# armadaproject/armada

Hardware: NVIDIA H100
Metric: job-placements/sec per scheduling round; 100k nodes x 1M jobs (higher is better)
Workload: dtype int64+f64

## Files before the change

### armada_b200/csrc/armada_dev.h

```cpp
#pragma once
#include <stdint.h>
#ifndef ARMADA_EMU
#include <vector_types.h>
#endif

#include "armada_b200.h"

#define ARMADA_DEV_MAX_QUEUES 128
#define ARMADA_DEV_MAX_SLOTS 22
#define ARMADA_DEV_VARIANTS (1 + ARMADA_MAX_AWAY)

struct DevCfg {
  int32_t D, R, PL, PC, Q, C, T, S, rows;
  uint32_t N, J, G;
  int32_t indexed_resource[ARMADA_MAX_RESOURCES];
  int64_t res_scale[ARMADA_MAX_RESOURCES];
  int32_t key_shift[ARMADA_MAX_RESOURCES];
  int32_t res_key_shift[ARMADA_MAX_RESOURCES];
  int32_t res_key_width[ARMADA_MAX_RESOURCES];
  int32_t node_bits;
  int32_t key_total_bits;
  int32_t key_width[ARMADA_MAX_RESOURCES];
  unsigned long long key_guard;
  int32_t swar_ok;
  int32_t cls_global;
  int32_t exact;
  int64_t index_res[ARMADA_MAX_RESOURCES];
  int32_t collect_excl;
  int32_t k32_ok;
  int32_t priorities[ARMADA_MAX_PRIORITIES];
  ArmadaPriorityClass pcs[ARMADA_MAX_PRIORITY_CLASSES];
  int64_t total_resources[ARMADA_MAX_RESOURCES];
  double drf_mult[ARMADA_MAX_RESOURCES];
  int64_t max_to_schedule[ARMADA_MAX_RESOURCES];
  uint8_t has_round_limit, protect_uncapped, prefer_large, disable_home, disable_away, disable_gang_away,
      global_inf, _pad;
  double protected_fraction;
  uint32_t max_lookback, disallowed_mask;
  double global_tokens;
  int64_t global_burst;
  int32_t max_slots, sw, tw;
  int32_t win_w;
  uint32_t off_cls, off_win, off_touched, off_slot, off_skey, off_srow, off_ssc, off_sgpos, off_hb_key, off_hb_row, off_hb_sc,
      off_ring, off_bt_k0, off_bt_k1, off_bt_id;
  int32_t bt_wq;
  int32_t bt_np;
  uint32_t uni_V;
  uint32_t floating_mask;
  int32_t floating_configured;
  int64_t floating_limit[ARMADA_MAX_RESOURCES];
};

struct DevPtrs {
  const int64_t* node_total;
  const int64_t* node_allocatable;
  const uint32_t* node_sclass;
  const uint8_t* node_flags;
  const int64_t* class_req_raw;
  const int64_t* class_req_node;
  const uint32_t* class_pc;
  const uint32_t* class_row;
  const uint8_t* class_key_valid;
  const double* class_cost;
  const uint4* q_rec;
  uint4* ev_rec;
  const uint32_t* static_match;
  unsigned char* cls_glob;
// ... 109 lines not shown
```

### armada_b200/csrc/armada_host.inc

```

#define CUDA_TRY(expr)                                                                     \
  do {                                                                                     \
    cudaError_t _e = (expr);                                                               \
    if (_e != cudaSuccess) {                                                               \
      g_last_error = std::string(#expr) + ": " + cudaGetErrorString(_e);                   \
      return ARMADA_E_CUDA;                                                                \
    }                                                                                      \
  } while (0)

#ifdef ARMADA_EMU
static std::recursive_mutex& emu_mutex() {
  static std::recursive_mutex m;
  return m;
}
#define ARMADA_EMU_SERIAL std::lock_guard<std::recursive_mutex> emu_lock_(emu_mutex())
#else
#define ARMADA_EMU_SERIAL ((void)0)
#endif

template <class T>
struct PinnedVec {
  T* p = nullptr;
  size_t n = 0, cap = 0;
  PinnedVec() = default;
// ... 579 lines not shown
    off = align16(off + 4 * S);
    cfg.bt_wq = 0;
    cfg.bt_np = 0;
    cfg.off_bt_k0 = cfg.off_bt_k1 = cfg.off_bt_id = (uint32_t)off;
    int wq_cap = exact ? 0 : 64;
    if (const char* e = getenv("ARMADA_BT_WQ"))
      if (!exact) wq_cap = std::max(8, atoi(e));
    for (int wq = 64; wq >= 8; wq >>= 1) {
      if ((size_t)wq * Q > 4096 || wq > wq_cap) continue;
      size_t np = 2;
      while (np < (size_t)wq * Q) np <<= 1;
      size_t need = 2 * (8 + 8 + 2 + 2) * np + 64;
      if (off + need + 16 <= (size_t)dev_smem) {
        cfg.bt_wq = wq;
        cfg.bt_np = (int32_t)np;
        cfg.off_bt_k0 = (uint32_t)off;
        cfg.off_bt_k1 = (uint32_t)(off + 8 * np);
        off = align16(off + 2 * 16 * np);
        cfg.off_bt_id = (uint32_t)off;
        off = align16(off + 2 * 2 * 2 * np);
        break;
      }
    }
    r->smem_bytes = off + 16;
    if (timing)
      fprintf(stderr,
              "smem layout: %zu bytes (header %zu, batch buffers at %u, %d items per queue per batch, np %d, %d slots)"
              " exact %d swar_ok %d k32_ok %d key_total_bits %d node_bits %d bt_wq %d\n",
              r->smem_bytes, sizeof(SmemHdr), cfg.off_bt_k0, cfg.bt_wq, cfg.bt_np, cfg.max_slots, cfg.exact, cfg.swar_ok, cfg.k32_ok,
              cfg.key_total_bits, cfg.node_bits, cfg.bt_wq);
    if (r->smem_bytes > (size_t)dev_smem) return fail_status(ARMADA_E_UNSUPPORTED, "shared-memory layout does not fit");
    CUDA_TRY(cudaFuncSetAttribute(k_schedule_pass<1>, cudaFuncAttributeMaxDynamicSharedMemorySize, dev_smem));
    CUDA_TRY(cudaFuncSetAttribute(k_schedule_pass<2>, cudaFuncAttributeMaxDynamicSharedMemorySize, dev_smem));
    CUDA_TRY(cudaFuncSetAttribute(k_schedule_pass<3>, cudaFuncAttributeMaxDynamicSharedMemorySize, dev_smem));
    CUDA_TRY(cudaFuncSetAttribute(k_schedule_pass<4>, cudaFuncAttributeMaxDynamicSharedMemorySize, dev_smem));
    CUDA_TRY(cudaFuncSetAttribute(k_schedule_pass<8>, cudaFuncAttributeMaxDynamicSharedMemorySize, dev_smem));
  }

  lap("domain+layout");
  r->node_perm.assign(N, 0);
  r->node_inv.assign(N, 0);
  for (uint32_t n = 0; n < N; ++n) {
    r->node_perm[in->node_id_rank[n]] = n;
    r->node_inv[n] = in->node_id_rank[n];
  }
  std::vector<int64_t> h_total((size_t)D * N), h_alloc((size_t)D * N);
  std::vector<uint32_t> h_sclass(N);
  std::vector<uint8_t> h_flags(N);
  for (uint32_t dn = 0; dn < N; ++dn) {
    uint32_t e = r->node_perm[dn];
    h_sclass[dn] = in->node_static_class[e];
    h_flags[dn] = in->node_flags[e];
    for (uint32_t d = 0; d < D; ++d) {
// ... 400 lines not shown
  DA(excl, cfg.collect_excl ? (size_t)J * ARMADA_EXCLUDED_KINDS : 16);
  DA(undo_log, 5 * (3 * (size_t)J + 16));
  DA(ev_rec, J);
  DA(fp_avail, (size_t)D * N);
  DA(fp_epoch, N);
  DA(fp_head, N);
  DA(fp_next, J);
  DA(fp_bad, N);
  DA(nl_start, (size_t)N + 1);
  DA(nl_item, J);
  DA(nl_pos, J);
  DA(nver, N);
  DA(fc_ver, 16 * (size_t)N);
  DA(bver, (N + 255) / 256 + 1);
  DA(fc_bver, 8 * ((size_t)(N + 255) / 256 + 1));
  DA(fc_bmax, 8 * ((size_t)(N + 255) / 256 + 1));
  DA(q_alloc, (size_t)Q * D);
  DA(q_alloc_pc, (size_t)Q * PC * D);
  DA(q_fair, (size_t)Q * 3);
  DA(q_tokens, Q);
  DA(s_scheduled, D);
  DA(s_evicted, D);
  DA(s_counts, 8);
  DA(stats, 48);
  {
    void* dp = nullptr;
    CUDA_TRY(cudaHostGetDevicePointer(&dp, r->h_dbg, 0));
    P.dbg_host = (uint32_t*)dp;
  }
  st = r->dalloc(&r->d_state, J);
  if (st) return st;
  st = r->dalloc(&r->d_method, J);
  if (st) return st;
  st = r->dalloc(&r->d_reason, J);
  if (st) return st;
  st = r->dalloc(&r->d_node, J);
  if (st) return st;
  st = r->dalloc(&r->d_sched_at, J);
  if (st) return st;
  st = r->dalloc(&r->d_preempted_at, J);
  if (st) return st;
  st = r->dalloc(&r->d_evict_queue, Q);
  if (st) return st;
  st = r->dalloc(&r->d_oversub, N);
  if (st) return st;
  st = r->dalloc(&r->d_hist, 256 * (size_t)grid_for(std::max<uint32_t>(std::max(J, N), 1), RS_THREADS * RS_ITEMS) + 1024);
  if (st) return st;
// ... 198 lines not shown
    CUDA_TRY(cudaEventRecord(r->evp[3], s));
    launches += 1;
  }
  ARMADA_LAUNCH(k_finalize, gj, 256, 0, s, c, P, r->d_state, r->d_node, r->d_sched_at, r->d_preempted_at, r->d_method, r->d_reason);
  launches += 1;
  CUDA_TRY(cudaEventRecord(r->ev1, s));
  CUDA_TRY(cudaGetLastError());
  {
    cudaError_t e = cudaStreamSynchronize(s);
    if (e != cudaSuccess) {
      std::string msg = std::string("cudaStreamSynchronize: ") + cudaGetErrorString(e);
      if (r->h_dbg && r->h_dbg[0]) {
        msg += "; device watchdog: spin loop " + std::to_string(r->h_dbg[0]) + " in warp " + std::to_string(r->h_dbg[1]) + " wr=" + std::to_string(r->h_dbg[3]) + " rd=";
        for (int i = 0; i < 12; ++i) msg += std::to_string(r->h_dbg[4 + i]) + ",";
        msg += " bt_prog=";
        for (int i = 0; i < 12; ++i) msg += std::to_string(r->h_dbg[20 + i]) + ",";
        msg += " pl_ready=" + std::to_string(r->h_dbg[36]) + " pl_chain=" + std::to_string(r->h_dbg[37]) + " pl_home=" + std::to_string(r->h_dbg[38]) + " iters=" + std::to_string(r->h_dbg[39]);
      }
      g_last_error = msg;
      return ARMADA_E_CUDA;
    }
  }
  long long counts[8];
  unsigned long long dstats[48];
  CUDA_TRY(cudaMemcpy(counts, P.s_counts, sizeof(counts), cudaMemcpyDeviceToHost));
  CUDA_TRY(cudaMemcpy(dstats, P.stats, sizeof(dstats), cudaMemcpyDeviceToHost));
  if (counts[5] == 100) return fail_status(ARMADA_E_DEADLINE, "the round did not finish within its time budget; nothing was committed");
  if (counts[5] != 0) return fail_status(ARMADA_E_INTERNAL, "device invariant violated, code " + std::to_string(counts[5]));
  float ms = 0;
  CUDA_TRY(cudaEventElapsedTime(&ms, r->ev0, r->ev1));
  r->stats = ArmadaRoundStats{};
  if (getenv("ARMADA_PRINT_STATS"))
    fprintf(stderr,
            "armada stats: kernel_cycles=%llu startup=%llu pipeline_runs=%llu chain_busy=%llu chain_wait=%llu epilogue=%llu precreate=%llu first_batch_wait=%llu "
            "after_chain_wait=%llu failed_iters=%llu failed_cycles=%llu fair_query_cycles=%llu level_scan_cycles=%llu evicted_rebind_cycles=%llu\n",
            dstats[5], dstats[6], dstats[7], dstats[24], dstats[25], dstats[16 + 7], dstats[32], dstats[33], dstats[34], dstats[35], dstats[36], dstats[37],
            dstats[38], dstats[39]);
  if (getenv("ARMADA_PRINT_STATS"))
    fprintf(stderr,
            "armada general loop: wait_index_warps=%llu ring_full=%llu select_queued=%llu (n=%llu) bind_queued=%llu fair_victims=%llu iteration_prologue=%llu\n",
            dstats[40], dstats[41], dstats[42], dstats[46], dstats[43], dstats[44], dstats[45]);
  r->stats.loop_iterations = dstats[0];
  r->stats.probes = dstats[1];
  r->stats.placements = dstats[2];
  r->stats.fair_preemption_scans = dstats[3];
  r->stats.tree_rescans = dstats[4];
  for (int i = 0; i < 8; ++i) r->stats.phase_cycles[i] = dstats[8 + i];
  for (int i = 0; i < 8; ++i) r->stats.batch_cycles[i] = dstats[16 + i];
  for (int i = 0; i < 8; ++i) r->stats.batch_debug[i] = dstats[24 + i];
  r->stats.evicted_pass1 = e1;
  r->stats.evicted_pass2 = e2;
  r->stats.gpu_launches = launches;
  r->stats.device_ms = ms;
  {
    float p1 = 0, p2 = 0;
    CUDA_TRY(cudaEventElapsedTime(&p1, r->evp[0], r->evp[1]));
    if (e2 > 0) CUDA_TRY(cudaEventElapsedTime(&p2, r->evp[2], r->evp[3]));
    r->stats.schedule_pass_ms = p1 + p2;
  }
  if (stats) *stats = r->stats;
  r->ran = true;
  return ARMADA_OK;
}

// ... 193 lines not shown
```

### armada_b200/csrc/armada_pass.inc

```

#define g_c (H->env_c)
#define g_p (H->env_p)
#define g_a (H->env_a)

#define PASS_WARPS 16
#define PASS_THREADS (PASS_WARPS * 32)
#define IDX_WARPS 15
#define CTL_WARP (PASS_WARPS - 1)
#define IDX_OWNERS (IDX_WARPS - 1)
#define WIN 32
#define WIN_TARGET 12
#define WIN_LOW 4
#define MSG_CAP 32
#define TLOG_CAP 32

enum { MSG_EXIT = 0, MSG_UPDATE0 = 1, MSG_NEWSLOT = 2, MSG_SCAN = 3, MSG_BATCH = 4, MSG_SUCC = 5, MSG_FAIR = 6 };
#define BT_RING 32

#define REC_EVICTED 0x80000000u
#define REC_GANG 0x40000000u
#define REC_QEV 0x20000000u
#define REC_GS 0x10000000u
#define REC_GSL 0x08000000u
#define REC_CLS_MASK 0x00FFFFFFu
// ... 127 lines not shown
  uint32_t bt_lim[2];
  uint32_t cmask[8];
  uint32_t sc_mask[32];
  uint32_t bt_lastpos[2][ARMADA_DEV_MAX_QUEUES];
  uint32_t bt_apc[2][ARMADA_DEV_MAX_QUEUES];
  uint32_t bt_njobs[2][ARMADA_DEV_MAX_QUEUES];
  uint32_t pl_extra;
  uint32_t pl_cut, pl_skip;
  uint4 gang_rec;
  uint32_t gang_cons[64];
  uint32_t bt_fh[ARMADA_DEV_MAX_SLOTS];
  uint32_t grp_of[32];
  uint32_t grp_diff[32];
  int grp_ns;
  unsigned long long t_runs;
  unsigned long long tl[8];
  uint32_t grp_resume[32];
  uint32_t grp_first[32];
  uint32_t bt_lazy;
  unsigned long long slot_preq[32];
  uint32_t slot_okp;
  unsigned long long slot_py[32];
  uint4 cand_scr[32];
  unsigned long long bt_fk[ARMADA_DEV_MAX_SLOTS];
  unsigned long long seq_base;
  uint32_t bt_cool, bt_cool_len, bt_batches;
  int bt_precreated;
  unsigned long long bt_cyc[8];
  unsigned long long bt_dbg[8];
  BtRes bt_ring[BT_RING];
  unsigned long long prof[8];
  int error;
  unsigned long long deadline_ns;
};

struct Views {
  ClassRec* cls;
  uint4* win;
  uint32_t* touched;
  SlotHdr* slot;
  unsigned long long* skey;
  int64_t* srow;
  uint32_t* ssc;
  uint32_t* sgpos;
  unsigned long long* hb_key;
  int64_t* hb_row;
  uint32_t* hb_sc;
  Msg* ring;
  unsigned long long* bt_k0;
  unsigned long long* bt_k1;
  uint16_t* bt_id;
};

__device__ __forceinline__ Views make_views(const DevCfg& c, unsigned char* smem_raw) {
  Views V;
  V.cls = c.cls_global ? (ClassRec*)((SmemHdr*)smem_raw)->env_p.cls_glob : (ClassRec*)(smem_raw + c.off_cls);
  V.win = (uint4*)(smem_raw + c.off_win);
  V.touched = (uint32_t*)(smem_raw + c.off_touched);
  V.slot = (SlotHdr*)(smem_raw + c.off_slot);
  V.skey = (unsigned long long*)(smem_raw + c.off_skey);
  V.srow = (int64_t*)(smem_raw + c.off_srow);
  V.ssc = (uint32_t*)(smem_raw + c.off_ssc);
  V.sgpos = (uint32_t*)(smem_raw + c.off_sgpos);
  V.hb_key = (unsigned long long*)(smem_raw + c.off_hb_key);
  V.hb_row = (int64_t*)(smem_raw + c.off_hb_row);
  V.hb_sc = (uint32_t*)(smem_raw + c.off_hb_sc);
  V.ring = (Msg*)(smem_raw + c.off_ring);
  V.bt_k0 = (unsigned long long*)(smem_raw + c.off_bt_k0);
  V.bt_k1 = (unsigned long long*)(smem_raw + c.off_bt_k1);
  V.bt_id = (uint16_t*)(smem_raw + c.off_bt_id);
  return V;
}

#ifdef ARMADA_EMU
#define ARMADA_SMEM_BASE (emu::M().dyn_smem)
#else
extern __shared__ __align__(16) unsigned char armada_smem[];
#define ARMADA_SMEM_BASE armada_smem
#endif
#define H ((SmemHdr*)ARMADA_SMEM_BASE)
#define V (make_views(g_c, ARMADA_SMEM_BASE))
#define nodemask ((1ull << g_c.node_bits) - 1ull)

#define DEXACT(DM) ((DM) <= 4)

#define PROF_BEGIN long long _t0 = clock64()
#define PROF_END(i)                                   \
  do {                                                \
    if (lane_id() == 0) H->prof[i] += clock64() - _t0; \
  } while (0)

__device__ __forceinline__ unsigned long long armada_now_ns() {
#ifdef ARMADA_EMU
// ... 207 lines not shown
        if (dg < sh.cursor) sh.cursor = dg;
        sh.wm = min_u64(sh.wm, dk);
      } else {
        sh.lostmin = min_u64(sh.lostmin, dk);
      }
    }
    __syncwarp();
  }

  static __device__ void update0(int s, uint32_t n, uint32_t sc, const int64_t* row) {
    SlotHdr& sh = V.slot[s];
    remove_node(s, n);
    bool fits = slot_static(sh, sc);
#pragma unroll
    for (int d = 0; d < DMAX; ++d)
      if (DEXACT(DMAX) || d < g_c.D) fits = fits && row[d] >= sh.req[d];
    if (!fits) return;
    unsigned long long dk;
    uint32_t dg;
    insert_entry(s, pack_key(g_c, row, n), row, sc, NONE, &dk, &dg);
    note_dropped(s, dk, dg);
  }

  static __device__ ARMADA_NOINLINE void cursor_chunk(int s, int max_take) {
    SlotHdr& sh = V.slot[s];
    const int l = lane_id();
    const uint32_t cur = sh.cursor;
    const uint32_t left = g_c.N - cur;
    int E = left < 32u ? (int)left : 32;
    if (E == 0) {
      __syncwarp();
      if (l == 0) sh.wm = KEY_INF;
      __syncwarp();
      return;
    }
    unsigned long long gk = KEY_INF;
    bool feas = false;
    int64_t r[DMAX];
    uint32_t sc = 0;
    if (g_c.swar_ok) {
      unsigned long long preq = 0;
      bool okp = true;
#pragma unroll
      for (int d = 0; d < DMAX; ++d)
        if (DEXACT(DMAX) || d < g_c.D) {
          okp = okp && (sh.req[d] >> g_c.res_key_width[d]) == 0;
          preq |= (unsigned long long)sh.req[d] << g_c.res_key_shift[d];
        }
      if (l < E) {
        gk = g_p.g0[cur + l];
        sc = g_p.g0_sc[cur + l];
        const uint32_t n = (uint32_t)(gk & nodemask);
        const bool touched = (V.touched[n >> 5] >> (n & 31)) & 1u;
        const unsigned long long G = g_c.key_guard;
        feas = !touched && okp && (gk >> g_c.key_total_bits) == 0 && slot_static(sh, sc) && ((((gk | G) - preq) & G) == G);
        if (feas) unpack_rows_t<DMAX>(g_c, gk, r);
      }
      if (cur + 32u + (uint32_t)l < g_c.N) {
        ARMADA_PREFETCH_L1(&g_p.g0[cur + 32u + (uint32_t)l]);
        ARMADA_PREFETCH_L1(&g_p.g0_sc[cur + 32u + (uint32_t)l]);
      }
    } else if (l < E) {
      gk = __ldcg(&g_p.g0[cur + l]);
      uint32_t n = (uint32_t)(gk & nodemask);
      bool touched = (V.touched[n >> 5] >> (n & 31)) & 1u;
      if (!touched) {
        sc = g_p.node_sclass[n];
        feas = slot_static(sh, sc);
#pragma unroll
        for (int d = 0; d < DMAX; ++d)
          if (DEXACT(DMAX) || d < g_c.D) {
            r[d] = __ldcg(&g_p.alloc[(size_t)d * g_c.N + n]);
            feas = feas && r[d] >= sh.req[d];
          }
      }
    }
    uint32_t m = __ballot_sync(FULL, feas);
    int taken = 0;
    {
      const uint32_t cntb = sh.cnt;
      const int nm = __popc(m);
// ... 28 lines not shown
#pragma unroll
      for (int d = 0; d < DMAX; ++d)
        if (DEXACT(DMAX) || d < g_c.D) row[d] = __shfl_sync(FULL, r[d], L);
      unsigned long long dk;
      uint32_t dg;
      insert_entry(s, key, row, esc, cur + (uint32_t)L, &dk, &dg);
      if (dk == key) {
        E = L;
        break;
      }
      note_dropped(s, dk, dg);
      ++taken;
    }
    unsigned long long edge = __shfl_sync(FULL, gk, E > 0 ? E - 1 : 0);
    unsigned long long stop_at = __shfl_sync(FULL, gk, E < 32 ? E : 31);
    __syncwarp();
    if (l == 0 && sh.cursor >= cur) {
      sh.cursor = cur + (uint32_t)E;
      if (sh.cursor >= g_c.N) sh.wm = KEY_INF;
      else if (E > 0) sh.wm = edge + 1;
      else sh.wm = stop_at;
    }
    __syncwarp();
  }

  static __device__ ARMADA_NOINLINE uint32_t g0_lower_bound(unsigned long long bound) {
    uint32_t lo = 0, hi = g_c.N;
    if (lane_id() == 0) {
      while (lo < hi) {
        uint32_t mid = (lo + hi) >> 1;
        if (__ldcg(&g_p.g0[mid]) < bound) lo = mid + 1;
        else hi = mid;
      }
    }
    return __shfl_sync(FULL, lo, 0);
  }

  static __device__ ARMADA_NOINLINE void scan_refill(int s, bool g0_valid) {
    SlotHdr& sh = V.slot[s];
    const int l = lane_id();
    request_fence();
    __syncwarp();
    if (l == 0) {
      sh.cnt = 0;
      atomicAdd(&H->st_rescans, 1ull);
    }
// ... 2478 lines not shown
      SlotHdr& sh = V.slot[s];
      const uint32_t cur = H->grp_resume[ld];
      __syncwarp();
      if (lane_id() == 0 && cur > sh.cursor) {
        sh.cnt = 0;
        sh.cursor = cur;
        sh.wm = cur < g_c.N ? g_p.g0[cur] : KEY_INF;
      }
      __syncwarp();
    }
    const BtRes* T = H->bt_ring;
    for (int j = 0; j < 32; ++j) {
      if (!T[j].flag) continue;
      int64_t row[DMAX];
#pragma unroll
      for (int d = 0; d < DMAX; ++d) row[d] = (DEXACT(DMAX) || d < g_c.D) ? T[j].row[d] : 0;
      Idx<DMAX>::update0(s, T[j].node, T[j].sc, row);
    }
    Idx<DMAX>::ensure_head(s, true);
  }

  static __device__ __forceinline__ void unpack_rows(unsigned long long key, int64_t* row) { unpack_rows_t<DMAX>(g_c, key, row); }

  static __device__ __forceinline__ uint32_t table_gc(bool valid, uint32_t sc, const int64_t* row) {
    const int ns = H->num_slots;
    bool alive = false;
    for (int s = 0; s < ns; ++s) {
      const SlotHdr& sh = V.slot[s];
      if (!sh.active) continue;
      bool f = valid && Idx<DMAX>::slot_static(sh, sc);
#pragma unroll
      for (int d = 0; d < DMAX; ++d)
        if (DEXACT(DMAX) || d < g_c.D) f = f && row[d] >= sh.req[d];
      alive = alive || f;
    }
    return __ballot_sync(FULL, alive);
  }

  template <bool K32>
  struct Lane {
    typename std::conditional<K32, uint32_t, unsigned long long>::type Y;
    uint32_t ck;
    uint32_t mystat, fullstat;
    uint32_t node;
  };
  static __device__ __forceinline__ uint32_t compact_of(unsigned long long key) {
    uint32_t c = 0;
    int cs = 0;
    for (int i = g_c.R - 1; i >= 0; --i) {
      c |= (uint32_t)((key >> g_c.key_shift[i]) & ((1ull << g_c.key_width[i]) - 1ull)) << cs;
      cs += g_c.key_width[i];
    }
    return c;
  }
  template <bool K32>
  static __device__ __forceinline__ void rerank(Lane<K32>& X) {
    uint32_t rank = 0;
    const uint32_t mine = X.fullstat != 0 ? X.node : NONE;
#pragma unroll
    for (int j = 0; j < 32; ++j) {
      const uint32_t nj = __shfl_sync(FULL, mine, j);
      if (nj < X.node) ++rank;
    }
    X.ck = (X.ck & ~0x3Eu) | ((rank & 31u) << 1);
  }
  template <bool K32>
  static __device__ __forceinline__ bool is_cand(const Lane<K32>& X) {
    return K32 ? (X.ck & 1u) != 0 && X.fullstat != 0 : (X.Y & 1) != 0;
  }
  template <bool K32>
  static __device__ __forceinline__ unsigned long long key_of(const Lane<K32>& X) {
    if (K32) return (((unsigned long long)X.Y << g_c.node_bits) & ~g_c.key_guard) | X.node;
    return ((unsigned long long)X.Y >> 1) & ~g_c.key_guard;
  }

  template <bool K32>
  static __device__ __forceinline__ bool install_body(Lane<K32>& X, uint32_t& have, uint32_t& exh, uint32_t s, int ns) {
    const int l = lane_id();
    const unsigned long long G = g_c.key_guard, nm = nodemask;
    const uint32_t sbit = 1u << s;
    BtRes* T = H->bt_ring;
    uint32_t fh = H->bt_fh[s], cnt = V.slot[s].cnt;
    unsigned long long e1 = KEY_INF;
    for (;;) {
      while (fh < cnt) {
        const unsigned long long k = V.skey[s * WIN + fh];
        const uint32_t en = (uint32_t)(k & nm);
        if (!((V.touched[en >> 5] >> (en & 31)) & 1u)) {
          e1 = k;
          break;
        }
        ++fh;
      }
      if (e1 != KEY_INF) break;
      if (V.slot[s].wm == KEY_INF) {
        have |= sbit;
        exh |= sbit;
        __syncwarp();
        if (l == 0) H->bt_fh[s] = fh;
        __syncwarp();
        return true;
      }
      __syncwarp();
      if (l == 0) V.slot[s].cnt = 0;
      __syncwarp();
      const long long tc0 = clock64();
      Idx<DMAX>::cursor_chunk((int)s, WIN);
      if (l == 0) {
        H->bt_dbg[6] += 1;
        H->bt_dbg[7] += (unsigned long long)(clock64() - tc0);
      }
      fh = 0;
      cnt = V.slot[s].cnt;
    }
    __syncwarp();
    if (l == 0) H->bt_fh[s] = fh;
    const uint32_t n1 = (uint32_t)(e1 & nm);
    const uint32_t dup = __ballot_sync(FULL, is_cand<K32>(X) && X.node == n1);
    if (dup) {
      if (l == __ffs(dup) - 1) X.mystat |= sbit;
      have |= sbit;
      return true;
    }
    uint32_t fm = ~__ballot_sync(FULL, X.fullstat != 0);
    if (!fm) {
      int64_t row[DMAX];
      unpack_rows(key_of<K32>(X), row);
      const bool cnd = is_cand<K32>(X);
      const uint32_t alive = table_gc(X.fullstat != 0 && !cnd, T[l].sc, row) | __ballot_sync(FULL, cnd);
      if (!((alive >> l) & 1u)) {
        X.Y = 0;
        X.ck = 0xFFFFFFFEu;
        X.mystat = X.fullstat = 0;
        X.node = NONE;
      }
      if (K32) rerank<K32>(X);
      fm = ~__ballot_sync(FULL, X.fullstat != 0);
      if (!fm) return false;
    }
    const int jf = __ffs(fm) - 1;
    const uint32_t nsc = V.ssc[s * WIN + fh];
    const uint32_t nstat = __ballot_sync(FULL, l < ns && V.slot[l < ns ? l : 0].active && Idx<DMAX>::slot_static(V.slot[l < ns ? l : 0], nsc));
    if (K32) {
      const uint32_t rnew = (uint32_t)__popc(__ballot_sync(FULL, X.fullstat != 0 && X.node < n1));
      if (X.fullstat != 0 && X.node > n1) X.ck += 2u;
      if (l == jf) X.ck = (compact_of(e1) << 6) | (rnew << 1) | 1u;
    }
    if (l == jf) {
      if (K32) X.Y = (uint32_t)((e1 | G) >> g_c.node_bits);
      else X.Y = ((e1 | G) << 1) | 1ull;
      X.mystat = sbit;
      X.fullstat = nstat;
      X.node = n1;
      T[jf].node = n1;
      T[jf].sc = nsc;
    }
    have |= sbit;
    return true;
  }
  template <bool K32>
  static __device__ ARMADA_NOINLINE bool install_general(Lane<K32>* Xp, uint32_t* havep, uint32_t* exhp, uint32_t s, int ns) {
    Lane<K32> X = *Xp;
    uint32_t have = *havep, exh = *exhp;
    const bool ok = install_body<K32>(X, have, exh, s, ns);
    *Xp = X;
    *havep = have;
    *exhp = exh;
    return ok;
  }
  static __device__ ARMADA_NOINLINE bool window_refill(uint32_t s) {
    const int l = lane_id();
    for (;;) {
      if (V.slot[s].wm == KEY_INF) {
        __syncwarp();
        if (l == 0) H->bt_fh[s] = V.slot[s].cnt;
        __syncwarp();
        return false;
      }
      __syncwarp();
      if (l == 0) V.slot[s].cnt = 0;
      __syncwarp();
      const long long tc0 = clock64();
      Idx<DMAX>::cursor_chunk((int)s, WIN);
      if (l == 0) {
        H->bt_dbg[6] += 1;
        H->bt_dbg[7] += (unsigned long long)(clock64() - tc0);
        H->bt_fh[s] = 0;
      }
      __syncwarp();
      if (V.slot[s].cnt > 0) return true;
    }
  }
  template <bool K32, class KT>
  static __device__ __forceinline__ int install_bulk(Lane<K32>& X, uint32_t& have, uint32_t s, int ns, const KT Gk) {
    const int l = lane_id();
    const unsigned long long G = g_c.key_guard, nm = nodemask;
    const uint32_t sbit = 1u << s;
    const uint32_t ltm = (1u << l) - 1u;
    const uint32_t fh = H->bt_fh[s], cnt = V.slot[s].cnt;
    const uint32_t pe = fh + (uint32_t)l;
    unsigned long long e = KEY_INF;
    uint32_t n = NONE, sc = 0, cke = 0;
    bool un = false;
    if (pe < cnt) {
      e = V.skey[s * WIN + pe];
      n = (uint32_t)(e & nm);
      un = !((V.touched[n >> 5] >> (n & 31)) & 1u);
      sc = V.ssc[s * WIN + pe];
      if (K32) {
        const uint32_t v = (uint32_t)(e >> g_c.node_bits);
        uint32_t c = 0;
#pragma unroll
        for (int k = 0; k < 8; ++k) c |= (v >> k) & H->cmask[k];
        cke = c << 6;
      }
    }
    const uint32_t um = __ballot_sync(FULL, un);
    if (!um) return 0;
    if (l == 0) H->bt_fh[s] = fh + (uint32_t)(__ffs(um) - 1);
    const bool cnd = is_cand<K32>(X);
    bool changed = false;
    uint32_t freem = ~__ballot_sync(FULL, X.fullstat != 0);
    if (__popc(freem) < 28) {
      bool alive = cnd;
      for (int t = 0; t < ns; ++t) {
        const KT py = (KT)H->slot_py[t];
        alive = alive || (((((KT)X.Y - py) & Gk) == Gk) && ((X.fullstat >> t) & 1u));
      }
      const uint32_t dead = __ballot_sync(FULL, X.fullstat != 0 && !alive);
      if (dead) {
        if ((dead >> l) & 1u) {
          X.Y = 0;
          X.ck = 0xFFFFFFFEu;
          X.mystat = X.fullstat = 0;
          X.node = NONE;
        }
        freem |= dead;
        changed = true;
      }
    }
    const int nfree = __popc(freem);
    int dupl = -1;
    {
      const uint32_t scm_e = __reduce_or_sync(FULL, (un && sc < 32u) ? 1u << sc : 0u);
      const uint32_t tsc = H->bt_ring[l].sc;
      const uint32_t scm_c = __reduce_or_sync(FULL, (cnd && tsc < 32u) ? 1u << tsc : 0u);
      const uint32_t big = __ballot_sync(FULL, (un && sc >= 32u) || (cnd && tsc >= 32u));
      if ((scm_e & scm_c) || big) {
        uint32_t cm = __ballot_sync(FULL, cnd);
        while (cm) {
          const int j = __ffs(cm) - 1;
          cm &= cm - 1;
          const uint32_t nj = __shfl_sync(FULL, X.node, j);
          if (un && nj == n) dupl = j;
        }
      }
    }
    const bool isnew = un && dupl < 0;
    const uint32_t newm = __ballot_sync(FULL, isnew);
    const int newrank = __popc(newm & ltm);
    const int maxnew = nfree > 3 ? nfree - 2 : nfree;
    const uint32_t stopm = __ballot_sync(FULL, un && ((isnew && newrank >= maxnew) || sc >= 32u));
    const uint32_t before = stopm ? ((1u << (__ffs(stopm) - 1)) - 1u) : 0xFFFFFFFFu;
    const bool take = un && ((before >> l) & 1u);
    const uint32_t takem = __ballot_sync(FULL, take);
    if (!takem) {
      if (changed && K32) rerank<K32>(X);
      return 2;
    }
    {
      uint32_t dm = __ballot_sync(FULL, take && dupl >= 0);
      while (dm) {
        const int i = __ffs(dm) - 1;
        dm &= dm - 1;
        const int j = __shfl_sync(FULL, dupl, i);
        if (l == j) X.mystat |= sbit;
      }
    }
    const int nnew = __popc(takem & newm);
    if (nnew) {
      uint4* scr = H->cand_scr;
      __syncwarp();
      if (take && isnew) scr[newrank] = make_uint4((uint32_t)e, (uint32_t)(e >> 32), sc, cke);
      __syncwarp();
      const int fr = __popc(freem & ltm);
      if (((freem >> l) & 1u) && fr < nnew) {
        const uint4 c = scr[fr];
        const unsigned long long e1 = ((unsigned long long)c.y << 32) | c.x;
        if (K32) {
          X.Y = (KT)((e1 | G) >> g_c.node_bits);
          X.ck = c.w | 1u;
        } else {
          X.Y = (KT)(((e1 | G) << 1) | 1ull);
        }
        X.mystat = sbit;
        X.fullstat = H->sc_mask[c.z];
        X.node = (uint32_t)(e1 & nm);
        H->bt_ring[l].node = X.node;
        H->bt_ring[l].sc = c.z;
      }
      __syncwarp();
    }
    if (K32 && (changed || nnew)) rerank<K32>(X);
    have |= sbit;
    return 1;
  }

  static __device__ __forceinline__ uint32_t warp_min_u32(uint32_t v) {
#ifdef ARMADA_EMU
    return __reduce_min_sync(FULL, v);
#else
    uint32_t m;
    asm volatile("redux.sync.min.u32 %0, %1, 0xffffffff;" : "=r"(m) : "r"(v));
    return m;
#endif
  }
  template <bool K32, class KT>
  static __device__ __forceinline__ int place(Lane<K32>& X, uint32_t& have, const uint32_t exh, const uint32_t lead, const KT Gk, const uint4 r, uint4* recp) {
    bool win, cand;
    uint32_t sbit;
    if (K32) {
      sbit = r.y;
      const uint32_t d = (uint32_t)X.Y - r.x;
      const bool fit = ((d & (uint32_t)Gk) == (uint32_t)Gk) && (X.mystat & sbit);
      const uint32_t m = warp_min_u32(fit ? X.ck : 0xFFFFFFFFu);
      if (m == 0xFFFFFFFFu) return 2;
// ... 73 lines not shown
      }
      if (t == total) return 0;
      if (mb == NOFIT) return 2;
      const bool wb = cka_post == mb;
      if (wb) {
        X.Y = Yb;
        if (K32) X.ck = (uint32_t)ckb;
        X.mystat = sw;
        rec[t].w = X.node;
      }
      ++t;
      if (mb & 1u) {
        if (wb) atomicOr(&V.touched[X.node >> 5], 1u << (X.node & 31));
        have = exh | __reduce_or_sync(FULL, is_cand<K32>(X) ? X.mystat : 0u);
        if (~have & lead) return 3;
      }
      if (t == total) return 0;
      ra = ran;
      rb = rbn;
    }
  }
  template <bool K32, class KT>
  static __device__ __forceinline__ bool ensure_groups(Lane<K32>& X, uint32_t& have, uint32_t& exh, const uint32_t lead, int ns, const KT Gk) {
    uint32_t need = ~have & lead;
    while (need) {
      const uint32_t s = (uint32_t)(__ffs(need) - 1);
      int r = install_bulk<K32, KT>(X, have, s, ns, Gk);
      if (r == 0) {
        if (!window_refill(s)) {
          have |= 1u << s;
          exh |= 1u << s;
          r = 1;
        } else {
          r = install_bulk<K32, KT>(X, have, s, ns, Gk);
        }
      }
      if (r != 1 && !install_general<K32>(&X, &have, &exh, s, ns)) return false;
      need = ~have & lead;
    }
    return true;
  }

  template <bool K32>
  static __device__ ARMADA_NOINLINE void chain_swar() {
    typedef typename std::conditional<K32, uint32_t, unsigned long long>::type KT;
    const int l = lane_id();
    {
      const long long tf0 = clock64();
      SPIN_BEGIN;
      while (Idx<DMAX>::uniform_ld(&H->pl_ready) == 0) {
        Ctl<DMAX>::service_fence();
        SPIN_CHECK(20);
        armada_emu_yield();
      }
      __threadfence_block();
      if (l == 0) H->tl[1] += (unsigned long long)(clock64() - tf0);
    }
    const int ns = H->num_slots;
    BtRes* T = H->bt_ring;
    const unsigned long long G = g_c.key_guard;
    KT Gk = K32 ? (KT)(G >> g_c.node_bits) : (KT)(G << 1);
#ifndef ARMADA_EMU
// ... 126 lines not shown
              break;
            }
            __syncwarp();
            const uint32_t nd = H->gang_rec.w;
            __syncwarp();
            if (l == 0) g_p.bt_gnode[((size_t)goff + t) * 64 + placed] = nd;
            const uint32_t gone = cm0 & ~__ballot_sync(FULL, is_cand<K32>(X));
            if (gone) {
              if (l == 0) H->gang_cons[ncons] = nd;
              ++ncons;
            }
            ++placed;
            if (c == 3 && !ensure_groups<K32, KT>(X, have, exh, lead, ns, Gk)) {
              failed = true;
              break;
            }
          }
          if (!failed) {
            if (limited && l < g_c.D) srun += (int64_t)card * V.cls[rec[t].z >> 8].req_raw[l];
            ++t;
            continue;
          }
          __syncwarp();
          if ((uint32_t)l < ncons) {
            const uint32_t nd = H->gang_cons[l];
            atomicAnd(&V.touched[nd >> 5], ~(1u << (nd & 31)));
          }
          X = Xs;
          H->bt_ring[l].node = X.node;
          H->bt_ring[l].sc = sc_s;
          {
            const unsigned long long* bk = reinterpret_cast<const unsigned long long*>(g_p.gang_bak);
            V.skey[s * WIN + l] = __ldcg(&bk[l]);
            const unsigned long long v = __ldcg(&bk[32 + l]);
            V.ssc[s * WIN + l] = (uint32_t)(v >> 32);
            V.sgpos[s * WIN + l] = (uint32_t)v;
            for (int d = 0; d < g_c.D; ++d) V.srow[(s * g_c.D + d) * WIN + l] = (int64_t)__ldcg(&bk[64 + d * 32 + l]);
          }
          if (l == 0) {
            V.slot[s].cnt = w_cnt;
            V.slot[s].cursor = w_cur;
            V.slot[s].wm = w_wm;
            V.slot[s].lostmin = w_lost;
            H->bt_fh[s] = w_fh;
          }
          __syncwarp();
// ... 493 lines not shown
    H->fence_req = H->fence_ack = 0;
    H->num_slots = 0;
    H->tcount = 0;
    H->num_unfeasible = 0;
    H->only_yield_evicted = 0;
    H->undo_n = 0;
    H->fp_epoch = 0;
    H->fc_n = H->fc_rr = 0;
    H->uni_slot = NONE;
    H->nl_valid = 0;
    H->ev_top = g_a.num_evicted;
    H->ov_with_queued = g_a.with_queued;
    H->ov_consider_priority = g_a.consider_priority;
    H->seq_base = g_p.stats[0];
    H->bt_cool = H->bt_cool_len = H->bt_batches = 0;
    H->bt_precreated = 0;
    H->grp_ns = -1;
    H->bt_lazy = 0;
    H->t_runs = 0;
    for (int i = 0; i < 8; ++i) H->tl[i] = 0;
    for (int i = 0; i < 8; ++i) H->gl[i] = 0;
    for (int i = 0; i < 32; ++i) H->grp_of[i] = (uint32_t)i;
    for (int i = 0; i < 8; ++i) H->bt_cyc[i] = H->bt_dbg[i] = 0;
    H->error = 0;
    H->deadline_ns = g_a.budget_ns ? armada_now_ns() + g_a.budget_ns : 0ull;
    H->st_iters = H->st_probes = H->st_placements = H->st_fair = H->st_rescans = 0;
    for (int i = 0; i < 8; ++i) H->prof[i] = 0;
    H->num_sched_jobs = g_p.s_counts[0];
    H->num_sched_gangs = g_p.s_counts[1];
    H->num_evicted_jobs = g_p.s_counts[2];
    H->global_tokens = __longlong_as_double(g_p.s_counts[4]);
    for (int d = 0; d < g_c.D; ++d) {
      H->s_scheduled[d] = g_p.s_scheduled[d];
      H->s_evicted[d] = g_p.s_evicted[d];
    }
  }
  if (threadIdx.x < PASS_WARPS) H->rd[threadIdx.x] = 0;
  for (int q = threadIdx.x; q < g_c.Q; q += blockDim.x) {
    for (int d = 0; d < g_c.D; ++d) H->q_allocp[q][d] = g_p.q_alloc[(size_t)q * g_c.D + d] + g_p.queue_penalty[(size_t)q * g_c.D + d];
    H->q_weight[q] = g_p.queue_weight[q];
    H->q_tokens[q] = g_p.q_tokens[q];
    H->q_burst[q] = g_p.queue_burst[q];
    H->q_inf[q] = g_p.queue_inf[q];
    H->q_cordoned[q] = g_p.queue_cordoned[q];
    H->q_budget[q] = __ddiv_rn(g_p.q_fair[q * 3 + 1], g_p.queue_weight[q]);
    H->q_key0[q] = H->q_key1[q] = 0;
// ... 171 lines not shown
  for (int q = lane_id(); q < g_c.Q; q += 32) {
    for (int d = 0; d < g_c.D; ++d) g_p.q_alloc[(size_t)q * g_c.D + d] = H->q_allocp[q][d] - g_p.queue_penalty[(size_t)q * g_c.D + d];
    g_p.q_tokens[q] = H->q_tokens[q];
  }
  if (lane_id() == 0) {
    for (int d = 0; d < g_c.D; ++d) {
      g_p.s_scheduled[d] = H->s_scheduled[d];
      g_p.s_evicted[d] = H->s_evicted[d];
    }
    g_p.s_counts[0] = H->num_sched_jobs;
    g_p.s_counts[1] = H->num_sched_gangs;
    g_p.s_counts[2] = H->num_evicted_jobs;
    if (g_a.pass == 1) g_p.s_counts[3] = term;
    g_p.s_counts[4] = __double_as_longlong(H->global_tokens);
    if (g_a.pass == 1 || H->error) g_p.s_counts[5] = H->error;
    g_p.stats[0] += H->st_iters;
    g_p.stats[1] += H->st_probes;
    g_p.stats[2] += H->st_placements;
    g_p.stats[3] += H->st_fair;
    g_p.stats[4] += H->st_rescans;
    for (int i = 0; i < 8; ++i) g_p.stats[8 + i] += H->prof[i];
    for (int i = 0; i < 8; ++i) g_p.stats[16 + i] += H->bt_cyc[i];
    for (int i = 0; i < 8; ++i) g_p.stats[24 + i] += H->bt_dbg[i];
    g_p.stats[5] += (unsigned long long)(clock64() - t_kernel);
    g_p.stats[6] += (unsigned long long)(t_loop0 - t_kernel);
    g_p.stats[7] += H->t_runs;
    for (int i = 0; i < 8; ++i) g_p.stats[32 + i] += H->tl[i];
    for (int i = 0; i < 8; ++i) g_p.stats[40 + i] += H->gl[i];
  }
  __syncwarp();
  bar_all();
}
```

### armada_b200/csrc/armada_round.cu

```cuda
#ifdef ARMADA_EMU
#include "cuda_emu.h"
#else
#include <cuda_runtime.h>
#define ARMADA_LAUNCH(kern, grid, block, smem, stream, ...) kern<<<(grid), (block), (smem), (stream)>>>(__VA_ARGS__)
#define ARMADA_DYN_SMEM(name) extern __shared__ __align__(16) unsigned char name[]
#define ARMADA_NAMED_BARRIER(id, count) asm volatile("bar.sync %0, %1;" ::"n"(id), "n"(count) : "memory")
static __device__ __forceinline__ void armada_emu_yield() {}
#define ARMADA_NOINLINE __noinline__
#define ARMADA_EMU_MARK(id) ((void)0)
#define ARMADA_PREFETCH_L1(p) asm volatile("prefetch.global.L1 [%0];" ::"l"(p))
#endif

#include <algorithm>
#include <atomic>
#include <memory>
#include <condition_variable>
#include <mutex>
#include <chrono>
#include <thread>
#include <type_traits>
#include <cmath>
#include <cstdio>
#include <cstring>
#include <numeric>
// ... 42 lines not shown
    P.sched_prio[j] = NOPRIO;
    P.q_successful[j] = P.q_unsuccessful[j] = P.q_rescheduled[j] = P.q_evicted[j] = P.q_reason[j] = 0;
    P.jc_evicted[j] = 0;
    uint32_t g = P.job_gang[j];
    P.jc_card[j] = g == NONE ? 1u : P.gang_card[g];
    P.assigned_node[j] = NONE;
    P.in_preempted[j] = P.in_scheduled[j] = P.in_sae[j] = P.ev_mark[j] = 0;
    P.has_pctx[j] = 0;
    P.res_node[j] = NONE;
    P.res_sched_at[j] = NOPRIO;
    P.res_preempted_at[j] = NOPRIO;
    P.res_method[j] = 0;
    P.res_seq[j] = 0;
    P.ev_index_of_job[j] = -1;
    P.ev_alive[j] = 0;
  }
  for (size_t g = i; g < c.G; g += stride) {
    P.gang_fill[g] = 0;
    P.gang_ev[g] = 0;
  }
  for (size_t n = i; n < c.N; n += stride) P.fp_epoch[n] = 0;
  for (size_t k = i; k < (size_t)c.C; k += stride) P.unfeasible[k] = 0;
  if (i < 16) P.counters[i] = 0;
  if (i < 48) P.stats[i] = 0;
}

__global__ void k_bind_running(DevCfg c, DevPtrs P) {
  size_t j = blockIdx.x * (size_t)blockDim.x + threadIdx.x;
  if (j >= c.J) return;
  uint32_t n = P.job_node0[j];
  if (n == NONE) return;
  uint32_t cls = P.job_class[j];
  uint32_t pc = P.class_pc[cls];
  int32_t pr = P.job_sap0[j];
  if (pr == NOPRIO) pr = c.pcs[pc].priority;
  int32_t cut = cutoff_for(c, pc, pr);
  for (int p = 0; p < c.PL; ++p) {
    if (c.priorities[p] > cut) continue;
    for (int d = 0; d < c.D; ++d) {
      int64_t r = P.class_req_node[(size_t)cls * c.D + d];
      if (r) atomic_add_i64(&P.alloc[((size_t)p * c.D + d) * c.N + n], -r);
    }
  }
  P.bound_node[j] = n;
  P.sched_prio[j] = pr;
}

// ... 427 lines not shown
```

Before: 37.39 million.

## Stage next cursor chunk in shared memory and replace shuffle loops with smem reads

Window refills in the batch path now load the next 32 index keys and static-class words into a per-slot shared-memory staging buffer. When the cursor advances exactly one chunk, the following refill reads from that buffer instead of global memory, and it replaces the earlier L1 prefetch. The rerank and duplicate-search loops now publish each lane's node to shared memory and read four at a time, instead of doing 32 warp shuffles. The change also adds skip-if-empty logic before install_bulk and a batch of new per-path counters. These counters add shared-memory stores and warp syncs on hot paths.

```diff
diff --git a/armada_b200/csrc/armada_dev.h b/armada_b200/csrc/armada_dev.h
--- a/armada_b200/csrc/armada_dev.h
+++ b/armada_b200/csrc/armada_dev.h
@@ -43,6 +43,8 @@
   int32_t win_w;
   uint32_t off_cls, off_win, off_touched, off_slot, off_skey, off_srow, off_ssc, off_sgpos, off_hb_key, off_hb_row, off_hb_sc,
       off_ring, off_bt_k0, off_bt_k1, off_bt_id;
+  uint32_t off_stg;
+  int32_t stg_slots;
   int32_t bt_wq;
   int32_t bt_np;
   uint32_t uni_V;
diff --git a/armada_b200/csrc/armada_host.inc b/armada_b200/csrc/armada_host.inc
--- a/armada_b200/csrc/armada_host.inc
+++ b/armada_b200/csrc/armada_host.inc
@@ -625,13 +625,21 @@
         break;
       }
     }
+    cfg.stg_slots = 0;
+    cfg.off_stg = (uint32_t)off;
+    if (cfg.bt_wq > 0 && cfg.swar_ok) {
+      const size_t per = 32 * (8 + 4);
+      const size_t left = (size_t)dev_smem > off + 16 ? (size_t)dev_smem - off - 16 : 0;
+      cfg.stg_slots = (int32_t)std::min<size_t>((size_t)cfg.max_slots, left / per);
+      off = align16(off + per * (size_t)cfg.stg_slots);
+    }
     r->smem_bytes = off + 16;
     if (timing)
       fprintf(stderr,
               "smem layout: %zu bytes (header %zu, batch buffers at %u, %d items per queue per batch, np %d, %d slots)"
-              " exact %d swar_ok %d k32_ok %d key_total_bits %d node_bits %d bt_wq %d\n",
+              " exact %d swar_ok %d k32_ok %d key_total_bits %d node_bits %d bt_wq %d stg_slots %d\n",
               r->smem_bytes, sizeof(SmemHdr), cfg.off_bt_k0, cfg.bt_wq, cfg.bt_np, cfg.max_slots, cfg.exact, cfg.swar_ok, cfg.k32_ok,
-              cfg.key_total_bits, cfg.node_bits, cfg.bt_wq);
+              cfg.key_total_bits, cfg.node_bits, cfg.bt_wq, cfg.stg_slots);
     if (r->smem_bytes > (size_t)dev_smem) return fail_status(ARMADA_E_UNSUPPORTED, "shared-memory layout does not fit");
     CUDA_TRY(cudaFuncSetAttribute(k_schedule_pass<1>, cudaFuncAttributeMaxDynamicSharedMemorySize, dev_smem));
     CUDA_TRY(cudaFuncSetAttribute(k_schedule_pass<2>, cudaFuncAttributeMaxDynamicSharedMemorySize, dev_smem));
@@ -1078,7 +1086,7 @@
   DA(s_scheduled, D);
   DA(s_evicted, D);
   DA(s_counts, 8);
-  DA(stats, 48);
+  DA(stats, 57);
   {
     void* dp = nullptr;
     CUDA_TRY(cudaHostGetDevicePointer(&dp, r->h_dbg, 0));
@@ -1323,7 +1331,7 @@
     }
   }
   long long counts[8];
-  unsigned long long dstats[48];
+  unsigned long long dstats[57];
   CUDA_TRY(cudaMemcpy(counts, P.s_counts, sizeof(counts), cudaMemcpyDeviceToHost));
   CUDA_TRY(cudaMemcpy(dstats, P.stats, sizeof(dstats), cudaMemcpyDeviceToHost));
   if (counts[5] == 100) return fail_status(ARMADA_E_DEADLINE, "the round did not finish within its time budget; nothing was committed");
@@ -1341,6 +1349,12 @@
     fprintf(stderr,
             "armada general loop: wait_index_warps=%llu ring_full=%llu select_queued=%llu (n=%llu) bind_queued=%llu fair_victims=%llu iteration_prologue=%llu\n",
             dstats[40], dstats[41], dstats[42], dstats[46], dstats[43], dstats[44], dstats[45]);
+  if (getenv("ARMADA_PRINT_STATS"))
+    fprintf(stderr,
+            "armada slow step: steps=%llu cycles=%llu refills=%llu refill_cycles=%llu install_bulk=%llu sweeps=%llu dup_searches=%llu "
+            "reranks=%llu installed=%llu install_general=%llu table_gc=%llu gang_rollbacks=%llu staged_hits=%llu\n",
+            dstats[28], dstats[29], dstats[30], dstats[31], dstats[48], dstats[49], dstats[50], dstats[51], dstats[52], dstats[53], dstats[54],
+            dstats[55], dstats[56]);
   r->stats.loop_iterations = dstats[0];
   r->stats.probes = dstats[1];
   r->stats.placements = dstats[2];
diff --git a/armada_b200/csrc/armada_pass.inc b/armada_b200/csrc/armada_pass.inc
--- a/armada_b200/csrc/armada_pass.inc
+++ b/armada_b200/csrc/armada_pass.inc
@@ -173,6 +173,9 @@
   uint32_t slot_okp;
   unsigned long long slot_py[32];
   uint4 cand_scr[32];
+  __align__(16) uint32_t lane_node[32];
+  unsigned long long ss_cnt[32];
+  uint32_t stg_pos[ARMADA_DEV_MAX_SLOTS];
   unsigned long long bt_fk[ARMADA_DEV_MAX_SLOTS];
   unsigned long long seq_base;
   uint32_t bt_cool, bt_cool_len, bt_batches;
@@ -201,6 +204,8 @@
   unsigned long long* bt_k0;
   unsigned long long* bt_k1;
   uint16_t* bt_id;
+  unsigned long long* stg_key;
+  uint32_t* stg_sc;
 };
 
 __device__ __forceinline__ Views make_views(const DevCfg& c, unsigned char* smem_raw) {
@@ -220,6 +225,8 @@
   V.bt_k0 = (unsigned long long*)(smem_raw + c.off_bt_k0);
   V.bt_k1 = (unsigned long long*)(smem_raw + c.off_bt_k1);
   V.bt_id = (uint16_t*)(smem_raw + c.off_bt_id);
+  V.stg_key = (unsigned long long*)(smem_raw + c.off_stg);
+  V.stg_sc = (uint32_t*)(smem_raw + c.off_stg + 8u * 32u * (uint32_t)c.stg_slots);
   return V;
 }
 
@@ -473,7 +480,7 @@
     note_dropped(s, dk, dg);
   }
 
-  static __device__ ARMADA_NOINLINE void cursor_chunk(int s, int max_take) {
+  static __device__ ARMADA_NOINLINE void cursor_chunk(int s, int max_take, bool stage = false) {
     SlotHdr& sh = V.slot[s];
     const int l = lane_id();
     const uint32_t cur = sh.cursor;
@@ -489,6 +496,14 @@
     bool feas = false;
     int64_t r[DMAX];
     uint32_t sc = 0;
+    stage = stage && g_c.swar_ok && s < g_c.stg_slots;
+    const bool hit = stage && H->stg_pos[s] == cur;
+    unsigned long long nk = 0;
+    uint32_t nsc = 0;
+    if (stage && cur + 32u + (uint32_t)l < g_c.N) {
+      nk = g_p.g0[cur + 32u + (uint32_t)l];
+      nsc = g_p.g0_sc[cur + 32u + (uint32_t)l];
+    }
     if (g_c.swar_ok) {
       unsigned long long preq = 0;
       bool okp = true;
@@ -499,15 +514,20 @@
           preq |= (unsigned long long)sh.req[d] << g_c.res_key_shift[d];
         }
       if (l < E) {
-        gk = g_p.g0[cur + l];
-        sc = g_p.g0_sc[cur + l];
+        if (hit) {
+          gk = V.stg_key[s * 32 + l];
+          sc = V.stg_sc[s * 32 + l];
+        } else {
+          gk = g_p.g0[cur + l];
+          sc = g_p.g0_sc[cur + l];
+        }
         const uint32_t n = (uint32_t)(gk & nodemask);
         const bool touched = (V.touched[n >> 5] >> (n & 31)) & 1u;
         const unsigned long long G = g_c.key_guard;
         feas = !touched && okp && (gk >> g_c.key_total_bits) == 0 && slot_static(sh, sc) && ((((gk | G) - preq) & G) == G);
         if (feas) unpack_rows_t<DMAX>(g_c, gk, r);
       }
-      if (cur + 32u + (uint32_t)l < g_c.N) {
+      if (!stage && cur + 32u + (uint32_t)l < g_c.N) {
         ARMADA_PREFETCH_L1(&g_p.g0[cur + 32u + (uint32_t)l]);
         ARMADA_PREFETCH_L1(&g_p.g0_sc[cur + 32u + (uint32_t)l]);
       }
@@ -582,6 +602,20 @@
       else sh.wm = stop_at;
     }
     __syncwarp();
+    if (stage) {
+      const uint32_t nc = sh.cursor;
+      const bool keep = nc == cur + 32u && nc < g_c.N;
+      if (keep && nc + (uint32_t)l < g_c.N) {
+        V.stg_key[s * 32 + l] = nk;
+        V.stg_sc[s * 32 + l] = nsc;
+      }
+      __syncwarp();
+      if (l == 0) {
+        H->stg_pos[s] = keep ? nc : NONE;
+        if (hit) H->ss_cnt[8] += 1;
+      }
+      __syncwarp();
+    }
   }
 
   static __device__ ARMADA_NOINLINE uint32_t g0_lower_bound(unsigned long long bound) {
@@ -3106,6 +3140,13 @@
 
   static __device__ __forceinline__ void unpack_rows(unsigned long long key, int64_t* row) { unpack_rows_t<DMAX>(g_c, key, row); }
 
+  static __device__ __forceinline__ void ss_bump(unsigned long long& a, int i, unsigned long long v = 1ull) { a += lane_id() == i ? v : 0ull; }
+  static __device__ __forceinline__ void ss_bump_smem(int i) {
+    __syncwarp();
+    if (lane_id() == 0) H->ss_cnt[i] += 1;
+    __syncwarp();
+  }
+
   static __device__ __forceinline__ uint32_t table_gc(bool valid, uint32_t sc, const int64_t* row) {
     const int ns = H->num_slots;
     bool alive = false;
@@ -3137,14 +3178,20 @@
     }
     return c;
   }
+  static __device__ __forceinline__ void lanes_publish(uint32_t v) {
+    __syncwarp();
+    H->lane_node[lane_id()] = v;
+    __syncwarp();
+  }
+  static __device__ __forceinline__ uint4 lanes_read4(int j) { return *reinterpret_cast<const uint4*>(&H->lane_node[j]); }
   template <bool K32>
   static __device__ __forceinline__ void rerank(Lane<K32>& X) {
+    lanes_publish(X.fullstat != 0 ? X.node : NONE);
     uint32_t rank = 0;
-    const uint32_t mine = X.fullstat != 0 ? X.node : NONE;
-#pragma unroll
-    for (int j = 0; j < 32; ++j) {
-      const uint32_t nj = __shfl_sync(FULL, mine, j);
-      if (nj < X.node) ++rank;
+#pragma unroll
+    for (int j = 0; j < 32; j += 4) {
+      const uint4 v = lanes_read4(j);
+      rank += (uint32_t)(v.x < X.node) + (uint32_t)(v.y < X.node) + (uint32_t)(v.z < X.node) + (uint32_t)(v.w < X.node);
     }
     X.ck = (X.ck & ~0x3Eu) | ((rank & 31u) << 1);
   }
@@ -3189,7 +3236,7 @@
       if (l == 0) V.slot[s].cnt = 0;
       __syncwarp();
       const long long tc0 = clock64();
-      Idx<DMAX>::cursor_chunk((int)s, WIN);
+      Idx<DMAX>::cursor_chunk((int)s, WIN, true);
       if (l == 0) {
         H->bt_dbg[6] += 1;
         H->bt_dbg[7] += (unsigned long long)(clock64() - tc0);
@@ -3208,6 +3255,7 @@
     }
     uint32_t fm = ~__ballot_sync(FULL, X.fullstat != 0);
     if (!fm) {
+      ss_bump_smem(6);
       int64_t row[DMAX];
       unpack_rows(key_of<K32>(X), row);
       const bool cnd = is_cand<K32>(X);
@@ -3244,6 +3292,7 @@
   }
   template <bool K32>
   static __device__ ARMADA_NOINLINE bool install_general(Lane<K32>* Xp, uint32_t* havep, uint32_t* exhp, uint32_t s, int ns) {
+    ss_bump_smem(5);
     Lane<K32> X = *Xp;
     uint32_t have = *havep, exh = *exhp;
     const bool ok = install_body<K32>(X, have, exh, s, ns);
@@ -3265,7 +3314,7 @@
       if (l == 0) V.slot[s].cnt = 0;
       __syncwarp();
       const long long tc0 = clock64();
-      Idx<DMAX>::cursor_chunk((int)s, WIN);
+      Idx<DMAX>::cursor_chunk((int)s, WIN, true);
       if (l == 0) {
         H->bt_dbg[6] += 1;
         H->bt_dbg[7] += (unsigned long long)(clock64() - tc0);
@@ -3276,7 +3325,7 @@
     }
   }
   template <bool K32, class KT>
-  static __device__ __forceinline__ int install_bulk(Lane<K32>& X, uint32_t& have, uint32_t s, int ns, const KT Gk) {
+  static __device__ __forceinline__ int install_bulk(Lane<K32>& X, uint32_t& have, uint32_t s, int ns, const KT Gk, unsigned long long& ssa) {
     const int l = lane_id();
     const unsigned long long G = g_c.key_guard, nm = nodemask;
     const uint32_t sbit = 1u << s;
@@ -3299,6 +3348,7 @@
         cke = c << 6;
       }
     }
+    ss_bump(ssa, 0);
     const uint32_t um = __ballot_sync(FULL, un);
     if (!um) return 0;
     if (l == 0) H->bt_fh[s] = fh + (uint32_t)(__ffs(um) - 1);
@@ -3306,10 +3356,12 @@
     bool changed = false;
     uint32_t freem = ~__ballot_sync(FULL, X.fullstat != 0);
     if (__popc(freem) < 28) {
+      ss_bump(ssa, 1);
       bool alive = cnd;
+#pragma unroll 4
       for (int t = 0; t < ns; ++t) {
         const KT py = (KT)H->slot_py[t];
-        alive = alive || (((((KT)X.Y - py) & Gk) == Gk) && ((X.fullstat >> t) & 1u));
+        alive |= ((((KT)X.Y - py) & Gk) == Gk) & (((X.fullstat >> t) & 1u) != 0);
       }
       const uint32_t dead = __ballot_sync(FULL, X.fullstat != 0 && !alive);
       if (dead) {
@@ -3331,12 +3383,17 @@
       const uint32_t scm_c = __reduce_or_sync(FULL, (cnd && tsc < 32u) ? 1u << tsc : 0u);
       const uint32_t big = __ballot_sync(FULL, (un && sc >= 32u) || (cnd && tsc >= 32u));
       if ((scm_e & scm_c) || big) {
-        uint32_t cm = __ballot_sync(FULL, cnd);
-        while (cm) {
-          const int j = __ffs(cm) - 1;
-          cm &= cm - 1;
-          const uint32_t nj = __shfl_sync(FULL, X.node, j);
-          if (un && nj == n) dupl = j;
+        ss_bump(ssa, 2);
+        lanes_publish(cnd ? X.node : NONE);
+        if (un) {
+#pragma unroll
+          for (int j = 0; j < 32; j += 4) {
+            const uint4 v = lanes_read4(j);
+            dupl = v.x == n ? j : dupl;
+            dupl = v.y == n ? j + 1 : dupl;
+            dupl = v.z == n ? j + 2 : dupl;
+            dupl = v.w == n ? j + 3 : dupl;
+          }
         }
       }
     }
@@ -3349,7 +3406,10 @@
     const bool take = un && ((before >> l) & 1u);
     const uint32_t takem = __ballot_sync(FULL, take);
     if (!takem) {
-      if (changed && K32) rerank<K32>(X);
+      if (changed && K32) {
+        ss_bump(ssa, 3);
+        rerank<K32>(X);
+      }
       return 2;
     }
     {
@@ -3363,6 +3423,7 @@
     }
     const int nnew = __popc(takem & newm);
     if (nnew) {
+      ss_bump(ssa, 4, (unsigned long long)nnew);
       uint4* scr = H->cand_scr;
       __syncwarp();
       if (take && isnew) scr[newrank] = make_uint4((uint32_t)e, (uint32_t)(e >> 32), sc, cke);
@@ -3385,7 +3446,10 @@
       }
       __syncwarp();
     }
-    if (K32 && (changed || nnew)) rerank<K32>(X);
+    if (K32 && (changed || nnew)) {
+      ss_bump(ssa, 3);
+      rerank<K32>(X);
+    }
     have |= sbit;
     return 1;
   }
@@ -3505,22 +3569,30 @@
   }
   template <bool K32, class KT>
   static __device__ __forceinline__ bool ensure_groups(Lane<K32>& X, uint32_t& have, uint32_t& exh, const uint32_t lead, int ns, const KT Gk) {
+    unsigned long long ssa = H->ss_cnt[lane_id()];
     uint32_t need = ~have & lead;
     while (need) {
       const uint32_t s = (uint32_t)(__ffs(need) - 1);
-      int r = install_bulk<K32, KT>(X, have, s, ns, Gk);
+      int r = H->bt_fh[s] < V.slot[s].cnt ? install_bulk<K32, KT>(X, have, s, ns, Gk, ssa) : 0;
       if (r == 0) {
         if (!window_refill(s)) {
           have |= 1u << s;
           exh |= 1u << s;
           r = 1;
         } else {
-          r = install_bulk<K32, KT>(X, have, s, ns, Gk);
-        }
-      }
-      if (r != 1 && !install_general<K32>(&X, &have, &exh, s, ns)) return false;
+          r = install_bulk<K32, KT>(X, have, s, ns, Gk, ssa);
+        }
+      }
+      if (r != 1) {
+        __syncwarp();
+        if (lane_id() < 5) H->ss_cnt[lane_id()] = ssa;
+        if (!install_general<K32>(&X, &have, &exh, s, ns)) return false;
+        ssa = H->ss_cnt[lane_id()];
+      }
       need = ~have & lead;
     }
+    __syncwarp();
+    if (lane_id() < 5) H->ss_cnt[lane_id()] = ssa;
     return true;
   }
 
@@ -3693,6 +3765,7 @@
             continue;
           }
           __syncwarp();
+          ss_bump_smem(7);
           if ((uint32_t)l < ncons) {
             const uint32_t nd = H->gang_cons[l];
             atomicAnd(&V.touched[nd >> 5], ~(1u << (nd & 31)));
@@ -4232,6 +4305,8 @@
     for (int i = 0; i < 8; ++i) H->gl[i] = 0;
     for (int i = 0; i < 32; ++i) H->grp_of[i] = (uint32_t)i;
     for (int i = 0; i < 8; ++i) H->bt_cyc[i] = H->bt_dbg[i] = 0;
+    for (int i = 0; i < 32; ++i) H->ss_cnt[i] = 0;
+    for (int i = 0; i < ARMADA_DEV_MAX_SLOTS; ++i) H->stg_pos[i] = NONE;
     H->error = 0;
     H->deadline_ns = g_a.budget_ns ? armada_now_ns() + g_a.budget_ns : 0ull;
     H->st_iters = H->st_probes = H->st_placements = H->st_fair = H->st_rescans = 0;
@@ -4449,6 +4524,7 @@
     for (int i = 0; i < 8; ++i) g_p.stats[8 + i] += H->prof[i];
     for (int i = 0; i < 8; ++i) g_p.stats[16 + i] += H->bt_cyc[i];
     for (int i = 0; i < 8; ++i) g_p.stats[24 + i] += H->bt_dbg[i];
+    for (int i = 0; i < 9; ++i) g_p.stats[48 + i] += H->ss_cnt[i];
     g_p.stats[5] += (unsigned long long)(clock64() - t_kernel);
     g_p.stats[6] += (unsigned long long)(t_loop0 - t_kernel);
     g_p.stats[7] += H->t_runs;
diff --git a/armada_b200/csrc/armada_round.cu b/armada_b200/csrc/armada_round.cu
--- a/armada_b200/csrc/armada_round.cu
+++ b/armada_b200/csrc/armada_round.cu
@@ -88,7 +88,7 @@
   for (size_t n = i; n < c.N; n += stride) P.fp_epoch[n] = 0;
   for (size_t k = i; k < (size_t)c.C; k += stride) P.unfeasible[k] = 0;
   if (i < 16) P.counters[i] = 0;
-  if (i < 48) P.stats[i] = 0;
+  if (i < 57) P.stats[i] = 0;
 }
 
 __global__ void k_bind_running(DevCfg c, DevPtrs P) {
```

After: 37.64 million, median of 6. No clear change (+0.7%).
